# cvg/nicer-slam

Hardware: AMD Instinct MI355X
Metric: rays/sec (fwd+bwd), one tracking iteration (higher is better)
Workload: dtype f32; 1 GPU; Replica room0 tracking iteration, 1024 rays x 128 samples (+640 sampler evaluations/ray), single MI355X, fp32 [BASELINE configs[1]]; rays_per_gpu=1024, samples_per_ray=128, sampler_evals_per_ray=640, global_rays=1024, engine=fused, param_grads=False, hip_graph=True, driver=KernelTracker, python_gc=off inside the timed regions (as timeit), ray_chunks=1, cache_prewarm_steps=100, cache_prewarm_batches=disjoint from the warm-up and timed batches, parallelism=single, rccl_ranks=0, full=False

## Files before the change

### nicer_slam_amd/csrc/colour_fwd_body.inc

```
    desync_simd_partners();
    const int lane = threadIdx.x & 63;
    const int h = lane >> 5;
    const uint32_t tile = blockIdx.x * 4 + (threadIdx.x >> 6);
    if (tile * 32 >= a.src.P) return;
    const bool wave_live = true;
    uint32_t pid = tile * 32 + (lane & 31);
    const bool live = pid < a.src.P;
    if (!live) pid = a.src.P - 1;
    const uint32_t q = point_of(a.src, pid);
    float x[3], z, dir[3];
    uint32_t ray;
    load_point(a.src, q, x, ray, z);
#pragma unroll
    for (int d = 0; d < 3; ++d) dir[d] = a.src.rays_d[ray * 3 + d];
    float in[COL_IN_STEPS];
    colour_inputs(a, geom, tile, q, lane, h, x, dir, in, false, wave_live);
    f32x16 a1[2], a2[2];
    float rgb[3];
    uint32_t masks[2] = {0u, 0u};
    colour_mlp<Seq, false>(nullptr, a.wp, lane, h, in, a1, a2, rgb, a.save ? masks : nullptr);
    if (live && h == 0) {
#pragma unroll
        for (int j = 0; j < 3; ++j) a.rgb[(size_t)q * 3 + j] = rgb[j];
    }
    if (a.save) {
        float* ext = save_ext(a.save, a.src.P, tile);
        ext[lane] = __uint_as_float(masks[0]);
        ext[64 + lane] = __uint_as_float(masks[1]);
        if (h == 0) {
#pragma unroll
            for (int j = 0; j < 3; ++j) ext[128 + 32 * j + (lane & 31)] = rgb[j];
        }
    }
```

### nicer_slam_amd/csrc/render_colour.hip

```cpp
#include <cstdlib>
#include "sdf_net.hpp"

namespace nsa {

constexpr int CL = 16, CC = 2;

struct ColPack {
    static constexpr int kHH = a_block_floats(2, HS);
    static constexpr int kW0 = 0;
    static constexpr int kB0 = kW0 + a_block_floats(2, COL_IN_STEPS);
    static constexpr int kW1 = kB0 + 64;
    static constexpr int kB1 = kW1 + kHH;
    static constexpr int kW2V = kB1 + 64;
    static constexpr int kB2 = kW2V + 3 * 64;
    static constexpr int kW1T = kB2 + 64;
    static constexpr int kW0T = kW1T + kHH;
    static constexpr int kTotal = kW0T + a_block_floats(5, HS);
};

constexpr int kColStage = 7680;
template <bool BWD>
struct ColOps {
    static constexpr int n = BWD ? 6 : 3;
    __host__ __device__ static constexpr StageOp op(int i) {
        return i == 0 ? StageOp{ColPack::kW0, 2, 9, 0, 5} : i == 1 ? StageOp{ColPack::kW0, 2, 9, 5, 4}
             : i == 2 ? StageOp{ColPack::kW1, 2, 4, 0, 4} : i == 3 ? StageOp{ColPack::kW1T, 2, 4, 0, 4}
             : i == 4 ? StageOp{ColPack::kW0T, 5, 4, 0, 2} : StageOp{ColPack::kW0T, 5, 4, 2, 2};
    }
};

template <bool MAP>
struct ColBwdOps {
    static constexpr int n = MAP ? 6 : 3;
    static constexpr int kRev = MAP ? 3 : 0;
    __host__ __device__ static constexpr StageOp op(int i) { return ColOps<true>::op(MAP ? i : i + 3); }
};

constexpr int kSaveTile = 4096, kSaveExt = 256;
__device__ __forceinline__ float* save_ext(float* save, uint32_t P, uint32_t tile) {
    return save + (size_t)((P + 31) / 32) * kSaveTile + (size_t)tile * kSaveExt;
}

__device__ __forceinline__ uint32_t relu_mask(const f32x16 (&a)[2]) {
    uint32_t m = 0;
#pragma unroll
    for (int t = 0; t < 2; ++t)
#pragma unroll
        for (int r = 0; r < 16; ++r) m |= a[t][r] > 0.0f ? (1u << (16 * t + r)) : 0u;
    return m;
}

struct ColourArgs {
    PointSrc src;
    const float* table;
    const float* wp;
    float divide_factor;
    const float* grad;
    const float* feat;
    float* rgb;
    float* save;
    int save_no_features;
    const float* g_rgb;
    float* g_feat;
    float* g_grad;
    float* g_x;
    float* g_dir;
    int grid_grad;
    float* g_table;
    float* emit;
    uint32_t emit_ld;
};

enum : int { CE_IN = 0, CE_H1 = 130, CE_H2 = 194, CE_AB1 = 258, CE_AB2 = 322, CE_OB = 386, CE_ROWS = 389 };

struct ColEmitter {
    float* base;
    uint32_t ld;
    bool live;
    __device__ __forceinline__ void slot(int region, int s, int h, float v) const {
        base[(size_t)(region + 2 * s + h) * ld] = live ? v : 0.0f;
    }
    __device__ __forceinline__ void hid(int region, int q, int h, float v) const {
        const int f = 32 * (q >> 4) + (q & 3) + 8 * ((q & 15) >> 2) + 4 * h;
        base[(size_t)(region + f) * ld] = live ? v : 0.0f;
    }
};

__device__ __forceinline__ void colour_level_out(const float (&v)[8][CC], const float (&w)[3], const float (&dw)[3], float scale,
                                                 bool inside, int jl, float (&in)[COL_IN_STEPS], float* sv, bool sv_features = true) {
    float f[CC];
    blend<3, CC>(v, w, f);
#pragma unroll
    for (int c = 0; c < CC; ++c) in[49 + jl * CC + c] = inside ? f[c] : 0.0f;
    if (sv) {
        if (sv_features) {
#pragma unroll
            for (int c = 0; c < CC; ++c) sv[(jl * CC + c) * 64] = in[49 + jl * CC + c];
        }
#pragma unroll
        for (int gd = 0; gd < 3; ++gd) {
            float jr[CC];
            jacobian_row<3, CC>(v, w, dw, scale, gd, jr);
#pragma unroll
            for (int c = 0; c < CC; ++c) sv[(16 + (jl * 3 + gd) * CC + c) * 64] = inside ? jr[c] : 0.0f;
        }
    }
}

__device__ __forceinline__ void colour_inputs(const ColourArgs& a, const GridGeom16& geom, uint32_t tile, uint32_t q, int lane,
                                              int h, const float (&x)[3], const float (&dir)[3], float (&in)[COL_IN_STEPS],
                                              bool from_save, bool wave_live) {
    const float* fsrc = a.feat + (size_t)tile * 32 * 64 + lane;
#pragma unroll
    for (int q = 0; q < HS; ++q) in[q] = fsrc[q * 64];
    float gr[3];
#pragma unroll
    for (int d = 0; d < 3; ++d) gr[d] = a.grad[(size_t)q * 3 + d];
    in[32] = h ? x[1] : x[0];
    in[33] = h ? dir[0] : x[2];
    in[34] = h ? dir[2] : dir[1];
    in[35] = h ? gr[1] : gr[0];
    in[36] = h ? 0.0f : gr[2];
#pragma unroll
    for (int j = 0; j < 6; ++j) {
        const int g0 = 2 * j, g1 = 2 * j + 1;
        const float da = h ? dir[g1 % 3] : dir[g0 % 3];
        const float sc = h ? (float)(1 << (g1 / 3)) : (float)(1 << (g0 / 3));
        sincos_f(da * sc, in[37 + 2 * j], in[38 + 2 * j]);
    }
    if (from_save) {
        const float* sv = a.save + (size_t)tile * 64 * 64 + lane;
#pragma unroll
        for (int q = 0; q < 16; ++q) in[49 + q] = sv[q * 64];
        return;
    }
    float u[3];
#pragma unroll
    for (int d = 0; d < 3; ++d) u[d] = to_unit(x[d], a.divide_factor);
    float* sv = (a.save && wave_live) ? a.save + (size_t)tile * 64 * 64 + lane : nullptr;
#pragma unroll
    for (int jl = 0; jl < CL / 2; ++jl) {
        const LevelGeom lg = geom.lv[2 * jl + h];
        uint32_t cell[3];
        float w[3], dw[3];
        const bool inside = locate<3>(u, lg.scale, cell, w, dw);
        float v[8][CC];
        gather_corners<3, CC>(a.table, lg, cell, v);
        colour_level_out(v, w, dw, lg.scale, inside, jl, in, sv, !a.save_no_features);
    }
}

template <class Seq, bool STAGED>
__device__ __forceinline__ void colour_mlp(float* stage, const float* __restrict__ wp, int lane, int h,
                                           const float (&in)[COL_IN_STEPS], f32x16 (&a1)[2], f32x16 (&a2)[2], float (&rgb)[3],
                                           uint32_t* masks = nullptr) {
    load_vec<2>(wp + ColPack::kB0, h, a1);
    if (STAGED) {
        const float m_in = abs_max<COL_IN_STEPS>(in);
        gemm_staged_part<Seq, kColStage, COL_IN_STEPS, 2, 0, 5, true, false>(stage, wp, 0, lane, in, a1, &m_in);
        gemm_staged_part<Seq, kColStage, COL_IN_STEPS, 2, 5, 4, false, true>(stage, wp, 1, lane, in, a1, &m_in);
    } else {
        gemm_op<COL_IN_STEPS, 2>(wp + ColPack::kW0, lane, in, a1);
    }
    const float m_h1 = acc_abs_max<2>(a1);
    float h1[HS];
#pragma unroll
    for (int t = 0; t < 2; ++t)
#pragma unroll
        for (int r = 0; r < 16; ++r) h1[16 * t + r] = relu_f(a1[t][r]);
    if (masks) masks[0] = relu_mask(a1);
    load_vec<2>(wp + ColPack::kB1, h, a2);
    if (STAGED) gemm_staged_part<Seq, kColStage, HS, 2, 0, 4>(stage, wp, 2, lane, h1, a2, &m_h1);
    else        gemm_op<HS, 2>(wp + ColPack::kW1, lane, h1, a2, &m_h1);
    if (masks) masks[1] = relu_mask(a2);
#pragma unroll
    for (int j = 0; j < 3; ++j) {
        f32x16 wv[2];
        load_vec<2>(wp + ColPack::kW2V + 64 * j, h, wv);
        float part = 0.0f;
#pragma unroll
        for (int t = 0; t < 2; ++t)
#pragma unroll
            for (int r = 0; r < 16; ++r) part = fmaf(relu_f(a2[t][r]), wv[t][r], part);
        const float o = xhalf_sum(part) + wp[ColPack::kB2 + j];
        rgb[j] = 1.0f / (1.0f + expf(-o));
    }
}

#ifndef NSA_OCC_COL_FWD
#define NSA_OCC_COL_FWD 4
#endif
__global__ __launch_bounds__(256, NSA_OCC_COL_FWD) void k_colour_fwd(ColourArgs a, GridGeom16 geom) {
    using Seq = ColOps<false>;
#include "colour_fwd_body.inc"
}

#ifdef NSA_X_TS
static __device__ unsigned long long* g_ts_c = nullptr;
#define CTS_BEGIN const unsigned long long ts_start = ts_now(); unsigned long long ts_prev = ts_start; \
    if ((threadIdx.x & 63) == 0) for (int i = 0; i < 16; ++i) nsa_ts_lds[threadIdx.x >> 6][i] = 0;
#define CTS_MARK(slot) { const unsigned long long t_ = ts_now(); ts_add(slot, t_ - ts_prev); ts_prev = t_; }
#define CTS_END { ts_add(15, ts_now() - ts_start); if (g_ts_c && (threadIdx.x & 63) == 0) { \
    unsigned long long* o_ = g_ts_c + ((size_t)blockIdx.x * (blockDim.x >> 6) + (threadIdx.x >> 6)) * 16; \
    for (int i = 0; i < 16; ++i) o_[i] = nsa_ts_lds[threadIdx.x >> 6][i]; } }
#else
#define CTS_BEGIN
#define CTS_MARK(slot)
#define CTS_END
#endif
template <bool MAP>
__global__ __launch_bounds__(256, 2) void k_colour_bwd(ColourArgs a, GridGeom16 geom) {
    using Seq = ColBwdOps<MAP>;
    __shared__ __attribute__((aligned(16))) float stage[2 * kColStage];
    CTS_BEGIN
#define NSA_BODY_NW 4
#include "colour_bwd_body.inc"
#undef NSA_BODY_NW
    CTS_MARK(11)
    CTS_END
}

}

#define NSA_SDFNET_AS_HEADER
#include "render_sdfnet.hip"
#undef NSA_SDFNET_AS_HEADER

namespace nsa {

#define NSA_CC_NW 4
#define NSA_BODY_NW NSA_CC_NW
__global__ __launch_bounds__(64 * NSA_CC_NW, 2) void k_colour_coarse_bwd(ColourArgs ca, GridGeom16 cgeom, SdfNetArgs sa, GridGeom16 sgeom) {
    __shared__ __attribute__((aligned(16))) float stage[2 * kStageFloats];
    static_assert(kStageFloats >= kColStage, "the colour phase stages its parts in the SDF kernel's buffers");
    {
        constexpr bool MAP = false;
        using Seq = ColBwdOps<false>;
        const ColourArgs& a = ca;
        const GridGeom16& geom = cgeom;
#include "colour_bwd_body.inc"
    }
    __syncthreads();
    {
        constexpr int L = 4, C = 8, NH = 1;
        constexpr bool MAP = false;
        using P = SdfPack<NH>;
        using Seq = SdfOps<NH, true>;
        const SdfNetArgs& a = sa;
        const GridGeom16& geom = sgeom;
#include "sdfnet_bwd_body.inc"
    }
}
#undef NSA_BODY_NW

}

#define NSA_COMPOSITE_AS_HEADER
#include "render_composite.hip"
#undef NSA_COMPOSITE_AS_HEADER

namespace nsa {

__global__ __launch_bounds__(256, NSA_OCC_COL_FWD) void k_colour_fwd_track(ColourArgs ca, GridGeom16 cgeom, CompositeArgs ta,
                                                                            const float* __restrict__ gt, float* __restrict__ ray_loss,
                                                                            float inv_n) {
    {
        using Seq = ColOps<false>;
        const ColourArgs& a = ca;
        const GridGeom16& geom = cgeom;
#include "colour_fwd_body.inc"
    }
    __syncthreads();
    if ((threadIdx.x >> 6) == 0) {
        const CompositeArgs& a = ta;
        const int lane = threadIdx.x & 63;
        const uint32_t ray = blockIdx.x;
#include "composite_track_body.inc"
    }
}

__global__ __launch_bounds__(256, NSA_OCC_COL_FWD) void k_colour_fwd_composite(ColourArgs ca, GridGeom16 cgeom, CompositeArgs ta) {
    {
        using Seq = ColOps<false>;
        const ColourArgs& a = ca;
        const GridGeom16& geom = cgeom;
#include "colour_fwd_body.inc"
    }
    __syncthreads();
    if ((threadIdx.x >> 6) == 0) {
        const CompositeArgs& a = ta;
        const int lane = threadIdx.x & 63;
        const uint32_t ray = blockIdx.x;
#include "composite_fwd_body.inc"
    }
}

}

#if defined(NSA_X_TS) && NSA_PIECES != 1
extern "C" int nsa_debug_set_ts_colour(unsigned long long* p) {
    return hipMemcpyToSymbol(HIP_SYMBOL(nsa::g_ts_c), &p, sizeof(p)) == hipSuccess ? 0 : 3;
}
#endif

#ifndef NSA_ENTRY
#define NSA_ENTRY(x) x
#endif
#include "bf16_entries.hpp"

extern "C" {

static int colour_common(const nsa_points_t* pts, const nsa_grid_t* grid, nsa::ColourArgs* a, nsa::GridGeom16* geom) {
    using namespace nsa;
    if (!pts || !grid) return NSA_EBADARG;
    if (pts->points || !pts->rays_o || !pts->rays_d || !pts->z_vals || pts->S == 0) return NSA_EBADARG;
    if (!(grid->L == 16 && grid->C == 2)) return NSA_EUNSUPPORTED_NET;
    if (int rc = make_grid_geom16(grid->offsets_host, grid->L, grid->S, grid->H, geom, grid->C)) return rc;
    a->src = PointSrc{pts->rays_o, pts->rays_d, pts->z_vals, nullptr, pts->P, pts->S, pts->order};
    a->table = grid->table;
    a->divide_factor = grid->divide_factor;
    return NSA_OK;
}

int NSA_ENTRY(nsa_colour_forward)(const nsa_points_t* pts, const nsa_grid_t* grid, const float* packed, const float* grad,
                       const float* feat_hl, float* rgb, float* save, nsa_stream_t stream) {
#if NSA_PIECES != 1
    if (grid && grid->precision == 1) return nsa_colour_forward_bf16(pts, grid, packed, grad, feat_hl, rgb, save, stream);
#endif
    using namespace nsa;
    if (!packed || !grad || !feat_hl || !rgb) return NSA_EBADARG;
    ColourArgs a{};
    GridGeom16 geom;
    if (int rc = colour_common(pts, grid, &a, &geom)) return rc;
    if (pts->P == 0) return NSA_OK;
    a.wp = packed; a.grad = grad; a.feat = feat_hl; a.rgb = rgb; a.save = save;
    const uint32_t tiles = (pts->P + 31) / 32;
    launch_begin();
    hipLaunchKernelGGL(k_colour_fwd, dim3((tiles + 3) / 4), dim3(256), 0, (hipStream_t)stream, a, geom);
    return launch_end();
}

int NSA_ENTRY(nsa_colour_forward_composite)(const nsa_points_t* pts, const nsa_grid_t* grid, const float* packed, const float* grad,
                                 const float* feat_hl, float* rgb, float* save, const float* sdf, const float* voxels,
                                 uint32_t voxel_res, float* weights, float* rgb_values, float* depth, float* nmap, float* entropy,
                                 nsa_stream_t stream) {
#if NSA_PIECES != 1
    if (grid && grid->precision == 1)
        return nsa_colour_forward_composite_bf16(pts, grid, packed, grad, feat_hl, rgb, save, sdf, voxels, voxel_res, weights, rgb_values,
                                                 depth, nmap, entropy, stream);
#endif
    using namespace nsa;
    if (!packed || !grad || !feat_hl || !rgb || !sdf || !voxels || !weights || !rgb_values || !depth || !nmap || !entropy)
        return NSA_EBADARG;
    ColourArgs a{};
    GridGeom16 geom;
    if (int rc = colour_common(pts, grid, &a, &geom)) return rc;
    if (pts->P == 0) return NSA_OK;
    if (pts->points || pts->order || pts->S != 128 || pts->P % 128 != 0) return NSA_EBADARG;
    a.wp = packed; a.grad = grad; a.feat = feat_hl; a.rgb = rgb; a.save = save;
    CompositeArgs t{};
    t.rays_o = pts->rays_o; t.rays_d = pts->rays_d; t.z_vals = pts->z_vals; t.sdf = sdf; t.rgb = rgb; t.grad = grad; t.voxels = voxels;
    t.voxel_res = voxel_res; t.R = pts->P / 128; t.S = 128;
    t.weights = weights; t.rgb_values = rgb_values; t.depth = depth; t.nmap = nmap; t.entropy = entropy;
    launch_begin();
    hipLaunchKernelGGL(k_colour_fwd_composite, dim3(pts->P / 128), dim3(256), 0, (hipStream_t)stream, a, geom, t);
    return launch_end();
}

int NSA_ENTRY(nsa_colour_forward_track)(const nsa_points_t* pts, const nsa_grid_t* grid, const float* packed, const float* grad,
                             const float* feat_hl, float* rgb, float* save, const float* sdf, const float* voxels, uint32_t voxel_res,
                             const float* gt, uint32_t n_total, float* rgb_values, float* ray_loss, float* g_sdf, float* g_rgb,
                             float* g_grad, nsa_stream_t stream) {
#if NSA_PIECES != 1
    if (grid && grid->precision == 1)
        return nsa_colour_forward_track_bf16(pts, grid, packed, grad, feat_hl, rgb, save, sdf, voxels, voxel_res, gt, n_total, rgb_values,
                                             ray_loss, g_sdf, g_rgb, g_grad, stream);
#endif
    using namespace nsa;
    if (!packed || !grad || !feat_hl || !rgb || !sdf || !voxels || !gt || !rgb_values || !ray_loss || !g_sdf || !g_rgb || !g_grad)
        return NSA_EBADARG;
    ColourArgs a{};
    GridGeom16 geom;
    if (int rc = colour_common(pts, grid, &a, &geom)) return rc;
    if (pts->P == 0) return NSA_OK;
    if (pts->points || pts->order || pts->S != 128 || pts->P % 128 != 0 || n_total < pts->P / 128) return NSA_EBADARG;
    a.wp = packed; a.grad = grad; a.feat = feat_hl; a.rgb = rgb; a.save = save;
#ifndef NSA_X_SAVE_FEATURES
    a.save_no_features = 1;
#endif
    CompositeArgs t{};
    t.rays_o = pts->rays_o; t.rays_d = pts->rays_d; t.z_vals = pts->z_vals; t.sdf = sdf; t.rgb = rgb; t.voxels = voxels;
    t.voxel_res = voxel_res; t.R = pts->P / 128; t.S = 128;
    t.rgb_values = rgb_values; t.g_sdf = g_sdf; t.g_rgb = g_rgb; t.g_grad = g_grad;
    launch_begin();
    hipLaunchKernelGGL(k_colour_fwd_track, dim3(pts->P / 128), dim3(256), 0, (hipStream_t)stream, a, geom, t, gt, ray_loss,
                       1.0f / (float)(3 * (uint64_t)n_total));
    return launch_end();
}

int NSA_ENTRY(nsa_colour_backward)(const nsa_points_t* pts, const nsa_grid_t* grid, const float* packed, const float* grad,
                        const float* feat_hl, const float* save, const float* g_rgb, int grid_grad, float* g_feat_hl,
                        float* g_grad, float* g_x, float* g_dir, nsa_stream_t stream) {
#if NSA_PIECES != 1
    if (grid && grid->precision == 1) return nsa_colour_backward_bf16(pts, grid, packed, grad, feat_hl, save, g_rgb, grid_grad, g_feat_hl, g_grad, g_x, g_dir, stream);
#endif
    using namespace nsa;
    if (!packed || !grad || !feat_hl || !save || !g_rgb || !g_feat_hl || !g_grad || !g_x || !g_dir) return NSA_EBADARG;
    ColourArgs a{};
    GridGeom16 geom;
    if (int rc = colour_common(pts, grid, &a, &geom)) return rc;
    if (pts->P == 0) return NSA_OK;
    a.wp = packed; a.grad = grad; a.feat = feat_hl; a.save = const_cast<float*>(save); a.g_rgb = g_rgb;
    a.g_feat = g_feat_hl; a.g_grad = g_grad; a.g_x = g_x; a.g_dir = g_dir; a.grid_grad = grid_grad;
    const uint32_t tiles = (pts->P + 31) / 32;
    launch_begin();
    hipLaunchKernelGGL(k_colour_bwd<false>, dim3((tiles + 3) / 4), dim3(256), 0, (hipStream_t)stream, a, geom);
    return launch_end();
}

int NSA_ENTRY(nsa_colour_coarse_backward)(const nsa_points_t* pts, const nsa_grid_t* grid, const float* packed, const float* grad,
                               const float* feat_hl, const float* save, const float* g_rgb, int grid_grad, float* g_feat_hl,
                               float* g_grad, float* g_x, float* g_dir, const nsa_grid_t* coarse, const float* packed_coarse,
                               const float* g_sdf, nsa_stream_t stream) {
#if NSA_PIECES != 1
    if (grid && coarse && grid->precision == 1 && coarse->precision == 1)
        return nsa_colour_coarse_backward_bf16(pts, grid, packed, grad, feat_hl, save, g_rgb, grid_grad, g_feat_hl, g_grad, g_x, g_dir, coarse,
                                               packed_coarse, g_sdf, stream);
#endif
    using namespace nsa;
    if (!packed || !grad || !feat_hl || !save || !g_rgb || !g_feat_hl || !g_grad || !g_x || !g_dir || !coarse || !packed_coarse)
        return NSA_EBADARG;
    if (grid->precision != coarse->precision) return NSA_EBADARG;
    if (coarse->tile == 16 || !(coarse->L == 4 && coarse->C == 8 && coarse->n_hidden == 1)) return NSA_EUNSUPPORTED_NET;
    ColourArgs a{};
    GridGeom16 geom, sgeom;
    if (int rc = colour_common(pts, grid, &a, &geom)) return rc;
    if (pts->P == 0) return NSA_OK;
    if (int rc = make_grid_geom16(coarse->offsets_host, coarse->L, coarse->S, coarse->H, &sgeom, coarse->C)) return rc;
    a.wp = packed; a.grad = grad; a.feat = feat_hl; a.save = const_cast<float*>(save); a.g_rgb = g_rgb;
    a.g_feat = g_feat_hl; a.g_grad = g_grad; a.g_x = g_x; a.g_dir = g_dir; a.grid_grad = grid_grad;
    SdfNetArgs sa{};
    sa.src = a.src;
    sa.table = coarse->table; sa.wp = packed_coarse; sa.divide_factor = coarse->divide_factor; sa.accumulate = 1;
    sa.g_sdf = g_sdf; sa.g_feat = g_feat_hl; sa.g_grad = g_grad; sa.g_x = g_x;
    const uint32_t tiles = (pts->P + 31) / 32;
    launch_begin();
    hipLaunchKernelGGL(k_colour_coarse_bwd, dim3((tiles + NSA_CC_NW - 1) / NSA_CC_NW), dim3(64 * NSA_CC_NW), 0, (hipStream_t)stream, a, geom, sa, sgeom);
    return launch_end();
}

int NSA_ENTRY(nsa_colour_backward_params)(const nsa_points_t* pts, const nsa_grid_t* grid, const float* packed, const float* grad,
                               const float* feat_hl, const float* save, const float* g_rgb, int grid_grad,
                               float* g_feat_hl, float* g_grad, float* g_x, float* g_dir, float* g_table, float* emit,
                               uint32_t emit_ld, nsa_stream_t stream) {
#if NSA_PIECES != 1
    if (grid && grid->precision == 1) return nsa_colour_backward_params_bf16(pts, grid, packed, grad, feat_hl, save, g_rgb, grid_grad, g_feat_hl, g_grad, g_x, g_dir, g_table, emit, emit_ld, stream);
#endif
    using namespace nsa;
    if (!packed || !grad || !feat_hl || !save || !g_rgb || !g_feat_hl || !g_grad || !g_x || !g_dir) return NSA_EBADARG;
    if (!g_table && !emit) return NSA_EBADARG;
    ColourArgs a{};
    GridGeom16 geom;
    if (int rc = colour_common(pts, grid, &a, &geom)) return rc;
    if (pts->P == 0) return NSA_OK;
    if (emit && emit_ld < ((pts->P + 31) / 32) * 32) return NSA_EBADARG;
    a.wp = packed; a.grad = grad; a.feat = feat_hl; a.save = const_cast<float*>(save); a.g_rgb = g_rgb;
    a.g_feat = g_feat_hl; a.g_grad = g_grad; a.g_x = g_x; a.g_dir = g_dir; a.grid_grad = grid_grad;
    a.g_table = g_table; a.emit = emit; a.emit_ld = emit_ld;
    const uint32_t tiles = (pts->P + 31) / 32;
    launch_begin();
    hipLaunchKernelGGL(k_colour_bwd<true>, dim3((tiles + 3) / 4), dim3(256), 0, (hipStream_t)stream, a, geom);
    return launch_end();
}

int NSA_ENTRY(nsa_colour_emit_rows)(void) { return nsa::CE_ROWS; }

}
```

Baseline: 1.991 million rays/s.

## Add persistent wave-specialized colour forward+composite pipeline kernel for tracking

```diff
diff --git a/nicer_slam_amd/csrc/colour_fwd_body.inc b/nicer_slam_amd/csrc/colour_fwd_body.inc
--- a/nicer_slam_amd/csrc/colour_fwd_body.inc
+++ b/nicer_slam_amd/csrc/colour_fwd_body.inc
@@ -15,10 +15,12 @@
     for (int d = 0; d < 3; ++d) dir[d] = a.src.rays_d[ray * 3 + d];
     float in[COL_IN_STEPS];
     colour_inputs(a, geom, tile, q, lane, h, x, dir, in, false, wave_live);
+    CFTS_MARK(4)
     f32x16 a1[2], a2[2];
     float rgb[3];
     uint32_t masks[2] = {0u, 0u};
     colour_mlp<Seq, false>(nullptr, a.wp, lane, h, in, a1, a2, rgb, a.save ? masks : nullptr);
+    CFTS_MARK(5)
     if (live && h == 0) {
 #pragma unroll
         for (int j = 0; j < 3; ++j) a.rgb[(size_t)q * 3 + j] = rgb[j];
diff --git a/nicer_slam_amd/csrc/render_colour.hip b/nicer_slam_amd/csrc/render_colour.hip
--- a/nicer_slam_amd/csrc/render_colour.hip
+++ b/nicer_slam_amd/csrc/render_colour.hip
@@ -107,6 +107,62 @@
     }
 }
 
+__device__ __forceinline__ void colour_inputs_plain(const ColourArgs& a, uint32_t tile, uint32_t q, int lane, int h,
+                                                    const float (&x)[3], const float (&dir)[3], float (&in)[COL_IN_STEPS]) {
+    const float* fsrc = a.feat + (size_t)tile * 32 * 64 + lane;
+#pragma unroll
+    for (int q = 0; q < HS; ++q) in[q] = fsrc[q * 64];
+    float gr[3];
+#pragma unroll
+    for (int d = 0; d < 3; ++d) gr[d] = a.grad[(size_t)q * 3 + d];
+    in[32] = h ? x[1] : x[0];
+    in[33] = h ? dir[0] : x[2];
+    in[34] = h ? dir[2] : dir[1];
+    in[35] = h ? gr[1] : gr[0];
+    in[36] = h ? 0.0f : gr[2];
+#pragma unroll
+    for (int j = 0; j < 6; ++j) {
+        const int g0 = 2 * j, g1 = 2 * j + 1;
+        const float da = h ? dir[g1 % 3] : dir[g0 % 3];
+        const float sc = h ? (float)(1 << (g1 / 3)) : (float)(1 << (g0 / 3));
+        sincos_f(da * sc, in[37 + 2 * j], in[38 + 2 * j]);
+    }
+}
+
+template <bool ALL_AHEAD = false>
+__device__ __forceinline__ void colour_inputs_grid(const ColourArgs& a, const GridGeom16& geom, uint32_t tile, int lane, int h,
+                                                   const float (&x)[3], float (&in)[COL_IN_STEPS], bool wave_live) {
+    float u[3];
+#pragma unroll
+    for (int d = 0; d < 3; ++d) u[d] = to_unit(x[d], a.divide_factor);
+    float* sv = (a.save && wave_live) ? a.save + (size_t)tile * 64 * 64 + lane : nullptr;
+    if constexpr (ALL_AHEAD) {
+        float w[CL / 2][3], dw[CL / 2][3], v[CL / 2][8][CC];
+        bool inside[CL / 2];
+#pragma unroll
+        for (int jl = 0; jl < CL / 2; ++jl) {
+            const LevelGeom lg = geom.lv[2 * jl + h];
+            uint32_t cell[3];
+            inside[jl] = locate<3>(u, lg.scale, cell, w[jl], dw[jl]);
+            gather_corners<3, CC>(a.table, lg, cell, v[jl]);
+        }
+#pragma unroll
+        for (int jl = 0; jl < CL / 2; ++jl)
+            colour_level_out(v[jl], w[jl], dw[jl], geom.lv[2 * jl + h].scale, inside[jl], jl, in, sv, !a.save_no_features);
+        return;
+    }
+#pragma unroll
+    for (int jl = 0; jl < CL / 2; ++jl) {
+        const LevelGeom lg = geom.lv[2 * jl + h];
+        uint32_t cell[3];
+        float w[3], dw[3];
+        const bool inside = locate<3>(u, lg.scale, cell, w, dw);
+        float v[8][CC];
+        gather_corners<3, CC>(a.table, lg, cell, v);
+        colour_level_out(v, w, dw, lg.scale, inside, jl, in, sv, !a.save_no_features);
+    }
+}
+
 __device__ __forceinline__ void colour_inputs(const ColourArgs& a, const GridGeom16& geom, uint32_t tile, uint32_t q, int lane,
                                               int h, const float (&x)[3], const float (&dir)[3], float (&in)[COL_IN_STEPS],
                                               bool from_save, bool wave_live) {
@@ -185,14 +241,6 @@
         const float o = xhalf_sum(part) + wp[ColPack::kB2 + j];
         rgb[j] = 1.0f / (1.0f + expf(-o));
     }
-}
-
-#ifndef NSA_OCC_COL_FWD
-#define NSA_OCC_COL_FWD 4
-#endif
-__global__ __launch_bounds__(256, NSA_OCC_COL_FWD) void k_colour_fwd(ColourArgs a, GridGeom16 geom) {
-    using Seq = ColOps<false>;
-#include "colour_fwd_body.inc"
 }
 
 #ifdef NSA_X_TS
@@ -208,6 +256,15 @@
 #define CTS_MARK(slot)
 #define CTS_END
 #endif
+#define CFTS_MARK(slot)
+#ifndef NSA_OCC_COL_FWD
+#define NSA_OCC_COL_FWD 4
+#endif
+__global__ __launch_bounds__(256, NSA_OCC_COL_FWD) void k_colour_fwd(ColourArgs a, GridGeom16 geom) {
+    using Seq = ColOps<false>;
+#include "colour_fwd_body.inc"
+}
+
 template <bool MAP>
 __global__ __launch_bounds__(256, 2) void k_colour_bwd(ColourArgs a, GridGeom16 geom) {
     using Seq = ColBwdOps<MAP>;
@@ -233,6 +290,7 @@
 __global__ __launch_bounds__(64 * NSA_CC_NW, 2) void k_colour_coarse_bwd(ColourArgs ca, GridGeom16 cgeom, SdfNetArgs sa, GridGeom16 sgeom) {
     __shared__ __attribute__((aligned(16))) float stage[2 * kStageFloats];
     static_assert(kStageFloats >= kColStage, "the colour phase stages its parts in the SDF kernel's buffers");
+    CTS_BEGIN
     {
         constexpr bool MAP = false;
         using Seq = ColBwdOps<false>;
@@ -264,6 +322,12 @@
 __global__ __launch_bounds__(256, NSA_OCC_COL_FWD) void k_colour_fwd_track(ColourArgs ca, GridGeom16 cgeom, CompositeArgs ta,
                                                                             const float* __restrict__ gt, float* __restrict__ ray_loss,
                                                                             float inv_n) {
+    CTS_BEGIN
+#ifdef NSA_X_TS
+#undef CFTS_MARK
+#define CFTS_MARK(slot) { CTS_MARK(slot) if ((threadIdx.x & 63) == 0) nsa_ts_lds[threadIdx.x >> 6][8 + slot] = ts_prev; }
+    if ((threadIdx.x & 63) == 0) nsa_ts_lds[threadIdx.x >> 6][11] = ts_start;
+#endif
     {
         using Seq = ColOps<false>;
         const ColourArgs& a = ca;
@@ -271,11 +335,91 @@
 #include "colour_fwd_body.inc"
     }
     __syncthreads();
+    CFTS_MARK(6)
     if ((threadIdx.x >> 6) == 0) {
         const CompositeArgs& a = ta;
         const int lane = threadIdx.x & 63;
         const uint32_t ray = blockIdx.x;
 #include "composite_track_body.inc"
+    }
+    CTS_MARK(7)
+    CTS_END
+#ifdef NSA_X_TS
+#undef CFTS_MARK
+#define CFTS_MARK(slot)
+#endif
+}
+
+constexpr int kPipeWaves = 8;
+__global__ __launch_bounds__(64 * kPipeWaves, 2) void k_colour_fwd_track_pipe(ColourArgs ca, GridGeom16 cgeom, CompositeArgs ta,
+                                                                               const float* __restrict__ gt,
+                                                                               float* __restrict__ ray_loss, float inv_n) {
+    __shared__ float hand[2][4][16][64];
+    const int lane0 = threadIdx.x & 63;
+    const int wave = __builtin_amdgcn_readfirstlane(threadIdx.x >> 6);
+    const bool gatherer = wave < 4;
+    const int w = wave & 3;
+    const uint32_t R = ta.R;
+    const uint32_t n_rays = blockIdx.x < R ? (R - blockIdx.x + gridDim.x - 1) / gridDim.x : 0u;
+    if (gatherer) __builtin_amdgcn_s_setprio(1);
+    else          __builtin_amdgcn_s_setprio(0);
+    for (uint32_t step = 0; step < n_rays + 2; ++step) {
+        int lane = lane0;
+        asm volatile("" : "+v"(lane));
+        const int h = lane >> 5;
+        if (gatherer) {
+            if (step < n_rays) {
+                const ColourArgs& a = ca;
+                const uint32_t tile = (blockIdx.x + step * gridDim.x) * 4 + w;
+                const uint32_t q = point_of(a.src, tile * 32 + (lane & 31));
+                float x[3], z;
+                uint32_t ray;
+                load_point(a.src, q, x, ray, z);
+                float in[COL_IN_STEPS];
+                colour_inputs_grid<true>(a, cgeom, tile, lane, h, x, in, true);
+#pragma unroll
+                for (int s = 0; s < 16; ++s) hand[step & 1][w][s][lane] = in[49 + s];
+            }
+        } else {
+            if (w == 0 && step >= 2) {
+                const CompositeArgs& a = ta;
+                const uint32_t ray = blockIdx.x + (step - 2) * gridDim.x;
+#include "composite_track_body.inc"
+            }
+            if (step >= 1 && step <= n_rays) {
+                using Seq = ColOps<false>;
+                const ColourArgs& a = ca;
+                const uint32_t tile = (blockIdx.x + (step - 1) * gridDim.x) * 4 + w;
+                const uint32_t q = point_of(a.src, tile * 32 + (lane & 31));
+                float x[3], z, dir[3];
+                uint32_t ray;
+                load_point(a.src, q, x, ray, z);
+#pragma unroll
+                for (int d = 0; d < 3; ++d) dir[d] = a.src.rays_d[ray * 3 + d];
+                float in[COL_IN_STEPS];
+                colour_inputs_plain(a, tile, q, lane, h, x, dir, in);
+#pragma unroll
+                for (int s = 0; s < 16; ++s) in[49 + s] = hand[(step - 1) & 1][w][s][lane];
+                f32x16 a1[2], a2[2];
+                float rgb[3];
+                uint32_t masks[2] = {0u, 0u};
+                colour_mlp<Seq, false>(nullptr, a.wp, lane, h, in, a1, a2, rgb, a.save ? masks : nullptr);
+                if (h == 0) {
+#pragma unroll
+                    for (int j = 0; j < 3; ++j) a.rgb[(size_t)q * 3 + j] = rgb[j];
+                }
+                if (a.save) {
+                    float* ext = save_ext(a.save, a.src.P, tile);
+                    ext[lane] = __uint_as_float(masks[0]);
+                    ext[64 + lane] = __uint_as_float(masks[1]);
+                    if (h == 0) {
+#pragma unroll
+                        for (int j = 0; j < 3; ++j) ext[128 + 32 * j + (lane & 31)] = rgb[j];
+                    }
+                }
+            }
+        }
+        __syncthreads();
     }
 }
 
@@ -309,6 +453,26 @@
 #include "bf16_entries.hpp"
 
 extern "C" {
+
+#if NSA_PIECES != 1
+static int colour_pipe_blocks() {
+    static int n[64] = {0};
+    int dev = 0;
+    if (hipGetDevice(&dev) != hipSuccess || dev < 0 || dev >= 64) return 256;
+    if (n[dev] == 0) {
+        int cus = 0;
+        n[dev] = (hipDeviceGetAttribute(&cus, hipDeviceAttributeMultiprocessorCount, dev) == hipSuccess && cus > 0) ? cus : 256;
+    }
+    return n[dev];
+}
+constexpr uint32_t kPipeMinRaysPerCu = 4;
+static bool colour_fwd_pipe(uint32_t R) {
+    const char* e = getenv("NSA_COLOUR_FWD_PIPE");
+    if (e && e[0] == '0') return false;
+    if (e && e[0] == '1') return true;
+    return R >= kPipeMinRaysPerCu * (uint32_t)colour_pipe_blocks();
+}
+#endif
 
 static int colour_common(const nsa_points_t* pts, const nsa_grid_t* grid, nsa::ColourArgs* a, nsa::GridGeom16* geom) {
     using namespace nsa;
@@ -392,9 +556,17 @@
     t.rays_o = pts->rays_o; t.rays_d = pts->rays_d; t.z_vals = pts->z_vals; t.sdf = sdf; t.rgb = rgb; t.voxels = voxels;
     t.voxel_res = voxel_res; t.R = pts->P / 128; t.S = 128;
     t.rgb_values = rgb_values; t.g_sdf = g_sdf; t.g_rgb = g_rgb; t.g_grad = g_grad;
+    const float inv_n = 1.0f / (float)(3 * (uint64_t)n_total);
     launch_begin();
-    hipLaunchKernelGGL(k_colour_fwd_track, dim3(pts->P / 128), dim3(256), 0, (hipStream_t)stream, a, geom, t, gt, ray_loss,
-                       1.0f / (float)(3 * (uint64_t)n_total));
+#if NSA_PIECES != 1
+    if (colour_fwd_pipe(t.R)) {
+        const uint32_t cap = (uint32_t)colour_pipe_blocks();
+        hipLaunchKernelGGL(k_colour_fwd_track_pipe, dim3(t.R < cap ? t.R : cap), dim3(64 * kPipeWaves), 0, (hipStream_t)stream, a, geom, t,
+                           gt, ray_loss, inv_n);
+        return launch_end();
+    }
+#endif
+    hipLaunchKernelGGL(k_colour_fwd_track, dim3(pts->P / 128), dim3(256), 0, (hipStream_t)stream, a, geom, t, gt, ray_loss, inv_n);
     return launch_end();
 }
 
```

Result: slower. 1.946 million rays/s (-2.2%).
